# mpkuse/rgbd_odometry

Measured on AMD Instinct MI355X. Metric: frame-pair aligns/sec (640x480, 4-lvl pyr), higher is better.
Workload: dtype f32

## Files before the change

### rgbd_odometry_amd/csrc/dvo_fused.hip

```cpp
#include "dvo_kernel_common.h"
#include "dvo_point_pk.h"
#include "dvo_palette.h"
#include "dvo_tiled_step.h"

#include <type_traits>

#ifndef DVO_WPE256
#define DVO_WPE256 2
#endif
#ifndef DVO_P4_DEPTH
#define DVO_P4_DEPTH(BLOCK) ((BLOCK) == 256 ? 3 : 2)
#endif

namespace dvo {

template <bool WITH_H, bool WITH_E2 = false>
struct Acc7T {
    static constexpr bool with_h = WITH_H, with_e2 = WITH_E2;
    double g[6];
    double e2;
    int nvis;
    double H[WITH_H ? 21 : 1];
    E2Limbs l;
};
typedef Acc7T<false> Acc7;

template <typename ACC>
DVO_DEV void acc7_zero(ACC &a) {
#pragma unroll
    for (int k = 0; k < 6; k++) a.g[k] = 0.0;
    a.e2 = 0.0;
    a.nvis = 0;
    if constexpr (ACC::with_h) {
#pragma unroll
        for (int k = 0; k < 21; k++) a.H[k] = 0.0;
    }
    if constexpr (ACC::with_e2) e2_limbs_zero(a.l);
}
template <typename ACC>
DVO_DEV void acc_h_add(ACC &a, const double *jwd, const double *Jd) {
#pragma unroll
    for (int i = 0; i < 6; i++)
#pragma unroll
        for (int j = i; j < 6; j++) a.H[i * 6 - (i * (i - 1)) / 2 + (j - i)] = fma(jwd[i], Jd[j], a.H[i * 6 - (i * (i - 1)) / 2 + (j - i)]);
}

enum { TEX_G16 = DVO_TEXMODE_GLOBAL16, TEX_L16 = DVO_TEXMODE_LDS16, TEX_P4 = DVO_TEXMODE_PAL4 };

struct TexSrc {
    const char *g16;
    unsigned tile_col_bytes;
    const char *l16;
    const char *p4;
    unsigned p4_col_bytes;
};

struct __attribute__((packed, aligned(4))) U3 { unsigned a, b, c; };

template <int TEX> struct Round2 {
    v2f xn, yn, zn;
    v4f t0, t1;
    bool vis0, vis1;
};
template <> struct Round2<TEX_P4> {
    v2f xn, yn, zn;
    U3 t0, t1;
};

typedef const __attribute__((address_space(3))) float lds_cfloat;
typedef const __attribute__((address_space(3))) v2f lds_cv2f;

DVO_DEV unsigned texel_byte_offset(int yy, int xx, unsigned tile_col_bytes ) {
    static_assert(DVO_TILE_Y_LOG2 == 2 && DVO_TILE_X_LOG2 == 1, "written for 4x2 tiles");
    return __umul24((unsigned)(xx >> 1), tile_col_bytes) + ((unsigned)yy << 5) - (((unsigned)yy & 3u) << 4) + (((unsigned)xx & 1u) << 6);
}

DVO_DEV unsigned p4_byte_offset(int yy, int xx, unsigned p4_col_bytes ) {
    static_assert(DVO_P4_ROWS == 6, "written for 6 interior rows per line");
    const unsigned ty = __umul24((unsigned)yy, 43691u) >> 18;
    return __umul24((unsigned)(xx >> 2), p4_col_bytes) + 128u  + (((unsigned)xx & 3u) << 5) + ((unsigned)yy << 2) + __umul24(ty, 104u);
}

struct LdsPoints {
    const uint2 *p;
    const unsigned *w4;
    const unsigned *g4;
    const unsigned *hdr;
};

template <bool LDS_SRC>
DVO_DEV void load_compact(const LdsPoints &lp, const uint2 *__restrict__ gpts, int j, unsigned &k, float &z) {
    const uint2 a = LDS_SRC ? lp.p[j] : gpts[j];
    k = a.x; z = __uint_as_float(a.y);
}

struct PointPf { uint2 p0, p1; unsigned h0, h1;  };

DVO_DEV unsigned pt4_header(const LdsPoints &lp, int i, int end) {
    const int chunk = __builtin_amdgcn_readfirstlane(min(i, end - 1)) >> 6;
    return lp.hdr[chunk];
}
struct PointPf4 { unsigned w0, w1; };

DVO_DEV uint2 stream_point(const uint2 *__restrict__ p) { return *p; }
DVO_DEV unsigned stream_word(const unsigned *__restrict__ p) { return *p; }
template <bool LDS_SRC, int TEX, bool PT4 = false, bool FULL = false>
DVO_DEV void round2_issue(const IterConst &c, const TexSrc &ts, const LdsPoints &lp, const uint2 *__restrict__ gpts,
                          int i0, int i1, int end, int step, PointPf &pf, Round2<TEX> &b, bool &any_odd, int &nvis) {
    const bool valid0 = FULL || i0 < end, valid1 = FULL || i1 < end;
    v2f xx, yy, Z;
    if constexpr (PT4) {
        unsigned w0, w1;
        if constexpr (LDS_SRC) {
            w0 = lp.w4[valid0 ? i0 : (end - 1)];
            w1 = lp.w4[valid1 ? i1 : (end - 1)];
        } else {
            w0 = pf.p0.x; w1 = pf.p1.x;
            pf.p0.x = stream_word(lp.g4 + min(i0 + step, end - 1));
            pf.p1.x = stream_word(lp.g4 + min(i1 + step, end - 1));
        }
        float x0, y0, z0, x1, y1, z1;
        const unsigned L00 = pf.h0, L01 = pf.h1;
        pf.h0 = pt4_header(lp, i0 + step, end);
        pf.h1 = pt4_header(lp, i1 + step, end);
        pt4_decode(c.nby, c.inv_nby, c.half_inv_nby, w0, L00, x0, y0, z0);
        pt4_decode(c.nby, c.inv_nby, c.half_inv_nby, w1, L01, x1, y1, z1);
        xx.x = x0; xx.y = x1; yy.x = y0; yy.y = y1; Z.x = z0; Z.y = z1;
    } else {
    unsigned k0, k1;
    float z0, z1;
    if constexpr (LDS_SRC) {
        const int j0 = valid0 ? i0 : (end - 1), j1 = valid1 ? i1 : (end - 1);
        load_compact<true>(lp, gpts, j0, k0, z0);
        load_compact<true>(lp, gpts, j1, k1, z1);
    } else {
        k0 = pf.p0.x; z0 = __uint_as_float(pf.p0.y);
        k1 = pf.p1.x; z1 = __uint_as_float(pf.p1.y);
        pf.p0 = stream_point(gpts + min(i0 + step, end - 1));
        pf.p1 = stream_point(gpts + min(i1 + step, end - 1));
    }
    xx.x = (float)(k0 & 0xffffu); xx.y = (float)(k1 & 0xffffu);
    yy.x = (float)(k0 >> 16);     yy.y = (float)(k1 >> 16);
    Z.x = z0; Z.y = z1;
    }
    const v2f X = (Z * (xx - c.pcx)) * c.pfx;
    const v2f Y = (Z * (yy - c.pcy)) * c.pfy;
    v2f xn, yn, zn, u, v;
    if constexpr (TEX == TEX_P4) {
        lanemask odd;
        project_point2m(c, X, Y, Z, xn, yn, zn, u, v, odd);
        any_odd |= (odd != 0ull);
        int px0, py0, px1, py1;
        const lanemask in0 = pixel_in_range_mask(u.x, c.cols, px0) & pixel_in_range_mask(v.x, c.rows, py0);
        const lanemask in1 = pixel_in_range_mask(u.y, c.cols, px1) & pixel_in_range_mask(v.y, c.rows, py1);
        const lanemask vis0 = FULL ? in0 : (in0 & mask_lt_i32(i0, end)), vis1 = FULL ? in1 : (in1 & mask_lt_i32(i1, end));
        b.xn = xn; b.yn = yn; b.zn = zn;
        nvis += __popcll(vis0) + __popcll(vis1);
        const unsigned o0 = select_or_zero(vis0, p4_byte_offset(py0, px0, ts.p4_col_bytes));
        const unsigned o1 = select_or_zero(vis1, p4_byte_offset(py1, px1, ts.p4_col_bytes));
        b.t0 = *reinterpret_cast<const U3 *>(ts.p4 + o0);
        b.t1 = *reinterpret_cast<const U3 *>(ts.p4 + o1);
    } else {
        bool odd0, odd1;
        project_point2(c, X, Y, Z, xn, yn, zn, u, v, odd0, odd1);
        any_odd |= (__builtin_amdgcn_ballot_w64(odd0 || odd1) != 0ull);
        int px0, py0, px1, py1;
        const bool inx0 = pixel_in_range(u.x, c.cols, px0), iny0 = pixel_in_range(v.x, c.rows, py0);
        const bool inx1 = pixel_in_range(u.y, c.cols, px1), iny1 = pixel_in_range(v.y, c.rows, py1);
        const bool vis0 = inx0 && iny0 && valid0;
        const bool vis1 = inx1 && iny1 && valid1;
        b.xn = xn; b.yn = yn; b.zn = zn;
        b.vis0 = vis0; b.vis1 = vis1;
        unsigned o0 = texel_byte_offset(py0, px0, ts.tile_col_bytes);
        unsigned o1 = texel_byte_offset(py1, px1, ts.tile_col_bytes);
        o0 = vis0 ? o0 : 0u;
        o1 = vis1 ? o1 : 0u;
        const char *base = (TEX == TEX_L16) ? ts.l16 : ts.g16;
        b.t0 = *reinterpret_cast<const v4f *>(base + o0);
        b.t1 = *reinterpret_cast<const v4f *>(base + o1);
    }
}

DVO_DEV unsigned lshl3_add(int d, unsigned c) {
    unsigned r;
    asm("v_lshl_add_u32 %0, %1, 3, %2" : "=v"(r) : "v"(d), "v"(c));
    return r;
}
template <unsigned PAL>
DVO_DEV void p4_decode2(const U3 &t0, const U3 &t1, v2f &dt, v2f &gx, v2f &gy, v2f &w) {
    const unsigned c0 = t0.b & 0xfff8u, c1 = t1.b & 0xfff8u;
    const v2f pw0 = *(lds_cv2f *)(size_t)(PAL + c0);
    const v2f pw1 = *(lds_cv2f *)(size_t)(PAL + c1);
    v2f pu, pd, pr, pl;
    pu.x = *(lds_cfloat *)(size_t)(PAL + (t0.a & 0xfff8u));
    pu.y = *(lds_cfloat *)(size_t)(PAL + (t1.a & 0xfff8u));
    pd.x = *(lds_cfloat *)(size_t)(PAL + (t0.c & 0xfff8u));
    pd.y = *(lds_cfloat *)(size_t)(PAL + (t1.c & 0xfff8u));
    pr.x = *(lds_cfloat *)(size_t)(PAL + lshl3_add(__builtin_amdgcn_sbfe((int)t0.b, 16, 8), c0));
    pr.y = *(lds_cfloat *)(size_t)(PAL + lshl3_add(__builtin_amdgcn_sbfe((int)t1.b, 16, 8), c1));
    pl.x = *(lds_cfloat *)(size_t)(PAL + lshl3_add(((int)t0.b) >> 24, c0));
    pl.y = *(lds_cfloat *)(size_t)(PAL + lshl3_add(((int)t1.b) >> 24, c1));
    dt.x = pw0.x; dt.y = pw1.x; w.x = pw0.y; w.y = pw1.y;
    gx = (pr - pl) * 0.5f;
    gy = (pd - pu) * 0.5f;
}

template <typename ACC>
DVO_DEV void acc7_add(ACC &a, const float *jw, const float *J, float eps) {
    const double e = (double)eps;
    double jwd[6];
#pragma unroll
    for (int k = 0; k < 6; k++) { jwd[k] = (double)jw[k]; a.g[k] = fma(jwd[k], e, a.g[k]); }
    a.e2 = fma(e, e, a.e2);
    if constexpr (ACC::with_e2) e2_limbs_add(a.l, eps);
    if constexpr (ACC::with_h) {
        double Jd[6];
#pragma unroll
        for (int k = 0; k < 6; k++) Jd[k] = (double)J[k];
        acc_h_add(a, jwd, Jd);
    }
}

DVO_DEV void iter_const_pose(IterConst &c, const float *Rf, const float *tf) {
    c.r[0] = uniform_f(Rf[0]); c.r[1] = uniform_f(Rf[1]); c.r[2] = uniform_f(Rf[2]);
    c.r[3] = uniform_f(Rf[3]); c.r[4] = uniform_f(Rf[4]); c.r[5] = uniform_f(Rf[5]);
    c.r[6] = uniform_f(Rf[6]); c.r[7] = uniform_f(Rf[7]); c.r[8] = uniform_f(Rf[8]);
    c.t[0] = uniform_f(tf[0]); c.t[1] = uniform_f(tf[1]); c.t[2] = uniform_f(tf[2]);
}

struct AccE2 {
    static constexpr bool with_h = false;
    E2Limbs l;
    int nvis;
};
DVO_DEV void acc7_add(AccE2 &a, const float *, const float *, float eps) { e2_limbs_add(a.l, eps); }

template <int TEX, unsigned PAL, typename ACC>
DVO_DEV void round2_compute(const IterConst &c, const Round2<TEX> &b, ACC &a) {
    v2f jw[6], J[6];
    float eps0, eps1;
    if constexpr (TEX == TEX_P4) {
        v2f dt, gx, gy, wt;
        p4_decode2<PAL>(b.t0, b.t1, dt, gx, gy, wt);
        eps0 = dt.x; eps1 = dt.y;
        jacobian_weighted2p(c, b.xn, b.yn, b.zn, gx, gy, wt, jw, ACC::with_h ? J : nullptr);
    } else {
        a.nvis += __popcll(__builtin_amdgcn_ballot_w64(b.vis0)) + __popcll(__builtin_amdgcn_ballot_w64(b.vis1));
        eps0 = b.vis0 ? b.t0.x : 0.0f; eps1 = b.vis1 ? b.t1.x : 0.0f;
        const float w0 = b.vis0 ? b.t0.w : 0.0f, w1 = b.vis1 ? b.t1.w : 0.0f;
        const float gx0 = b.vis0 ? b.t0.y : 0.0f, gx1 = b.vis1 ? b.t1.y : 0.0f;
        const float gy0 = b.vis0 ? b.t0.z : 0.0f, gy1 = b.vis1 ? b.t1.z : 0.0f;
        jacobian_weighted2(c, b.xn, b.yn, b.zn, gx0, gx1, gy0, gy1, w0, w1, jw, ACC::with_h ? J : nullptr);
    }
    const double e0 = (double)eps0, e1 = (double)eps1;
    if constexpr (ACC::with_e2) { e2_limbs_add(a.l, eps0); e2_limbs_add(a.l, eps1); }
    if constexpr (!ACC::with_h) {
#pragma unroll
        for (int k = 0; k < 6; k++) {
            a.g[k] = fma((double)jw[k].x, e0, a.g[k]);
            a.g[k] = fma((double)jw[k].y, e1, a.g[k]);
        }
        a.e2 = fma(e0, e0, a.e2);
        a.e2 = fma(e1, e1, a.e2);
    } else {
        {
            double jd[6], Jd[6];
#pragma unroll
            for (int k = 0; k < 6; k++) { jd[k] = (double)jw[k].x; Jd[k] = (double)J[k].x; a.g[k] = fma(jd[k], e0, a.g[k]); }
            a.e2 = fma(e0, e0, a.e2);
            acc_h_add(a, jd, Jd);
        }
        __builtin_amdgcn_sched_barrier(0);
        {
            double jd[6], Jd[6];
#pragma unroll
            for (int k = 0; k < 6; k++) { jd[k] = (double)jw[k].y; Jd[k] = (double)J[k].y; a.g[k] = fma(jd[k], e1, a.g[k]); }
            a.e2 = fma(e1, e1, a.e2);
            acc_h_add(a, jd, Jd);
        }
        __builtin_amdgcn_sched_barrier(0);
    }
}

template <int BLOCK, bool LDS_SRC, int TEX, int DEPTH = 2, unsigned PAL = 0, bool PT4 = false, typename ACC = Acc7>
DVO_DEV void accumulate_points2(const IterConst &c, const TexSrc &ts, const LdsPoints &lp, const uint2 *__restrict__ gpts,
                                int first, int end, int lane_off, ACC &a, bool &any_odd) {
    if (first >= end) return;
    constexpr int STEP = 2 * BLOCK;
    const int wave_off = __builtin_amdgcn_readfirstlane(lane_off - (int)(threadIdx.x & 63));
    const int n_rounds = (end - first - wave_off + STEP - 1) / STEP;
    if (n_rounds <= 0) return;
#define DVO_ISSUE(buf, k) round2_issue<LDS_SRC, TEX, PT4>(c, ts, lp, gpts, base + (k) * STEP, base + (k) * STEP + BLOCK, end, STEP, pf, buf, any_odd, a.nvis)
#define DVO_ISSUE_FULL(buf, k) round2_issue<LDS_SRC, TEX, PT4, true>(c, ts, lp, gpts, base + (k) * STEP, base + (k) * STEP + BLOCK, end, STEP, pf, buf, any_odd, a.nvis)
#define DVO_COMPUTE(buf) round2_compute<TEX, PAL, ACC>(c, buf, a)
    int base = first + lane_off;
    PointPf pf;
    if constexpr (PT4) { pf.h0 = pt4_header(lp, base, end); pf.h1 = pt4_header(lp, base + BLOCK, end); }
    if constexpr (!LDS_SRC) {
        if constexpr (PT4) { pf.p0.x = stream_word(lp.g4 + min(base, end - 1)); pf.p1.x = stream_word(lp.g4 + min(base + BLOCK, end - 1)); }
        else { pf.p0 = stream_point(gpts + min(base, end - 1)); pf.p1 = stream_point(gpts + min(base + BLOCK, end - 1)); }
    }
    if constexpr (DEPTH == 3) {
        Round2<TEX> A, B, C;
        DVO_ISSUE(A, 0);
        if (n_rounds > 1) DVO_ISSUE(B, 1);
        int r = 0;
        for (; r + 4 < n_rounds; r += 3) {
            DVO_ISSUE_FULL(C, 2); DVO_COMPUTE(A);
            DVO_ISSUE_FULL(A, 3); DVO_COMPUTE(B);
            DVO_ISSUE(B, 4); DVO_COMPUTE(C);
            base += 3 * STEP;
        }
        const int left = n_rounds - r;
        if (left >= 3) DVO_ISSUE(C, 2);
        DVO_COMPUTE(A);
        if (left >= 2) {
            if (left >= 4) DVO_ISSUE(A, 3);
            DVO_COMPUTE(B);
            if (left >= 3) {
                DVO_COMPUTE(C);
                if (left >= 4) DVO_COMPUTE(A);
            }
        }
    } else {
        Round2<TEX> A, B;
        DVO_ISSUE(A, 0);
        int r = 0;
        for (; r + 2 < n_rounds; r += 2) {
            DVO_ISSUE_FULL(B, 1); DVO_COMPUTE(A);
            DVO_ISSUE(A, 2); DVO_COMPUTE(B);
            base += 2 * STEP;
        }
        if (r + 1 < n_rounds) {
            DVO_ISSUE(B, 1);
            DVO_COMPUTE(A);
            DVO_COMPUTE(B);
        } else {
            DVO_COMPUTE(A);
        }
    }
#undef DVO_ISSUE
#undef DVO_ISSUE_FULL
#undef DVO_COMPUTE
}

DVO_DEV float4 p4_texel(const TexSrc &ts, const float2 *pal_lds, int yy, int xx) {
    const U3 w = *reinterpret_cast<const U3 *>(ts.p4 + p4_byte_offset(yy, xx, ts.p4_col_bytes));
    const int c = (int)((w.b >> 3) & 0x1fffu);
    const int cr = c + __builtin_amdgcn_sbfe((int)w.b, 16, 8), cl = c + (((int)w.b) >> 24);
    const float2 pc = pal_lds[c];
    const float pr = pal_lds[cr].x, pl = pal_lds[cl].x, pu = pal_lds[(w.a >> 3) & 0x1fffu].x, pd = pal_lds[(w.c >> 3) & 0x1fffu].x;
    return make_float4(pc.x, (pr - pl) * 0.5f, (pd - pu) * 0.5f, pc.y);
}

template <int BLOCK, bool LDS_SRC, bool P4, bool PT4 = false, typename ACC = Acc7>
DVO_DEV void accumulate_points_exact(const IterConst &c, const char *__restrict__ tex, const TexSrc &ts, const float2 *pal_lds,
                                     const LdsPoints &lp, const uint2 *__restrict__ gpts, int first, int end, int lane_off, ACC &a) {
    for (int i = first + lane_off; __builtin_amdgcn_ballot_w64(i < end) != 0ull; i += BLOCK) {
        const bool valid = i < end;
        float X, Y, Z, xn, yn, zn, u, v;
        if constexpr (PT4) {
            const int j = valid ? i : (end - 1);
            const unsigned w = LDS_SRC ? lp.w4[j] : lp.g4[j];
            float xf, yf;
            pt4_decode(c.nby, c.inv_nby, c.half_inv_nby, w, pt4_header(lp, i, end), xf, yf, Z);
            X = Z * (xf - c.pcx) * c.pfx;
            Y = Z * (yf - c.pcy) * c.pfy;
        } else {
        unsigned k; float z;
        load_compact<LDS_SRC>(lp, gpts, valid ? i : (end - 1), k, z);
        expand_compact(c, k, z, X, Y, Z);
        }
        const bool vis = project_point(c, X, Y, Z, xn, yn, zn, u, v) && valid;
        a.nvis += __popcll(__builtin_amdgcn_ballot_w64(vis));
        if (vis) {
            const float4 t = P4 ? p4_texel(ts, pal_lds, (int)v, (int)u)
                                : reinterpret_cast<const float4 *>(tex)[texel_index((int)v, (int)u, c.tiles_per_col)];
            float J[6], jw[6];
            jacobian_row(c, xn, yn, zn, t.y, t.z, J);
#pragma unroll
            for (int q = 0; q < 6; q++) jw[q] = J[q] * t.w;
            acc7_add(a, jw, J, t.x);
        }
    }
}

template <int BLOCK, typename ACC>
DVO_DEV void sweep_literal(int mode, bool p4_partial, bool pt4, const IterConst &c, const char *__restrict__ tex, const TexSrc &ts, const float2 *pal_lds,
                           const LdsPoints &lp, const uint2 *__restrict__ gpts, int n_lds, int N, int lane_off, ACC &a) {
    if (mode == DVO_TEXMODE_PAL4 && p4_partial && pt4) {
        accumulate_points_exact<BLOCK, true, false, true, ACC>(c, tex, ts, pal_lds, lp, gpts, 0, n_lds, lane_off, a);
        accumulate_points_exact<BLOCK, false, false, true, ACC>(c, tex, ts, pal_lds, lp, gpts, n_lds, N, lane_off, a);
    } else if (mode == DVO_TEXMODE_PAL4 && p4_partial) {
        accumulate_points_exact<BLOCK, true, false, false, ACC>(c, tex, ts, pal_lds, lp, gpts, 0, n_lds, lane_off, a);
        accumulate_points_exact<BLOCK, false, false, false, ACC>(c, tex, ts, pal_lds, lp, gpts, n_lds, N, lane_off, a);
    } else if (mode == DVO_TEXMODE_PAL4 && pt4) {
        accumulate_points_exact<BLOCK, true, true, true, ACC>(c, tex, ts, pal_lds, lp, gpts, 0, n_lds, lane_off, a);
        accumulate_points_exact<BLOCK, false, true, true, ACC>(c, tex, ts, pal_lds, lp, gpts, n_lds, N, lane_off, a);
    } else if (mode == DVO_TEXMODE_PAL4) {
        accumulate_points_exact<BLOCK, true, true, false, ACC>(c, tex, ts, pal_lds, lp, gpts, 0, n_lds, lane_off, a);
        accumulate_points_exact<BLOCK, false, true, false, ACC>(c, tex, ts, pal_lds, lp, gpts, n_lds, N, lane_off, a);
    } else {
        accumulate_points_exact<BLOCK, true, false, false, ACC>(c, tex, ts, pal_lds, lp, gpts, 0, n_lds, lane_off, a);
        accumulate_points_exact<BLOCK, false, false, false, ACC>(c, tex, ts, pal_lds, lp, gpts, n_lds, N, lane_off, a);
    }
}

struct Final2 {
    v2f u, v, zn;
    unsigned w0, w1;
    bool vis0, vis1;
};
template <bool LDS_SRC, int TEX, bool PT4 = false>
DVO_DEV void final2_issue(const IterConst &c, const TexSrc &ts, const LdsPoints &lp, const uint2 *__restrict__ gpts,
                          int i0, int i1, int end, int step, PointPf &pf, Final2 &b) {
    float X0, Y0, Z0, X1, Y1, Z1;
    if constexpr (PT4) {
        unsigned w0, w1;
        if constexpr (LDS_SRC) {
            w0 = lp.w4[min(i0, end - 1)]; w1 = lp.w4[min(i1, end - 1)];
        } else {
            w0 = pf.p0.x; w1 = pf.p1.x;
            pf.p0.x = stream_word(lp.g4 + min(i0 + step, end - 1));
            pf.p1.x = stream_word(lp.g4 + min(i1 + step, end - 1));
        }
        float xf, yf;
        pt4_decode(c.nby, c.inv_nby, c.half_inv_nby, w0, pt4_header(lp, i0, end), xf, yf, Z0);
        X0 = Z0 * (xf - c.pcx) * c.pfx; Y0 = Z0 * (yf - c.pcy) * c.pfy;
        pt4_decode(c.nby, c.inv_nby, c.half_inv_nby, w1, pt4_header(lp, i1, end), xf, yf, Z1);
        X1 = Z1 * (xf - c.pcx) * c.pfx; Y1 = Z1 * (yf - c.pcy) * c.pfy;
    } else {
        unsigned k0, k1;
        float z0, z1;
        if constexpr (LDS_SRC) {
            load_compact<true>(lp, gpts, min(i0, end - 1), k0, z0);
            load_compact<true>(lp, gpts, min(i1, end - 1), k1, z1);
        } else {
            k0 = pf.p0.x; z0 = __uint_as_float(pf.p0.y);
            k1 = pf.p1.x; z1 = __uint_as_float(pf.p1.y);
            pf.p0 = stream_point(gpts + min(i0 + step, end - 1));
            pf.p1 = stream_point(gpts + min(i1 + step, end - 1));
        }
        expand_compact(c, k0, z0, X0, Y0, Z0);
        expand_compact(c, k1, z1, X1, Y1, Z1);
    }
    {
        float xs, ys, zs, us, vs;
        project_point(c, X0, Y0, Z0, xs, ys, zs, us, vs);
        b.u.x = us; b.v.x = vs; b.zn.x = zs;
        project_point(c, X1, Y1, Z1, xs, ys, zs, us, vs);
        b.u.y = us; b.v.y = vs; b.zn.y = zs;
    }
    int px0, py0, px1, py1;
    const bool inx0 = pixel_in_range(b.u.x, c.cols, px0), iny0 = pixel_in_range(b.v.x, c.rows, py0);
    const bool inx1 = pixel_in_range(b.u.y, c.cols, px1), iny1 = pixel_in_range(b.v.y, c.rows, py1);
    b.vis0 = inx0 && iny0; b.vis1 = inx1 && iny1;
    if constexpr (TEX == TEX_P4) {
        const unsigned o0 = b.vis0 ? p4_byte_offset(py0, px0, ts.p4_col_bytes) + 4u : 0u;
        const unsigned o1 = b.vis1 ? p4_byte_offset(py1, px1, ts.p4_col_bytes) + 4u : 0u;
        b.w0 = *reinterpret_cast<const unsigned *>(ts.p4 + o0);
        b.w1 = *reinterpret_cast<const unsigned *>(ts.p4 + o1);
    } else {
        const unsigned o0 = b.vis0 ? texel_byte_offset(py0, px0, ts.tile_col_bytes) : 0u;
        const unsigned o1 = b.vis1 ? texel_byte_offset(py1, px1, ts.tile_col_bytes) : 0u;
        const char *base = (TEX == TEX_L16) ? ts.l16 : ts.g16;
        b.w0 = *reinterpret_cast<const unsigned *>(base + o0);
        b.w1 = *reinterpret_cast<const unsigned *>(base + o1);
    }
}
template <int TEX, unsigned PAL>
DVO_DEV void final2_store(const Final2 &b, int i0, int i1, int end, float *__restrict__ fe, float *__restrict__ fr, const TexSrc &ts, bool partial) {
    float e0, e1;
    if constexpr (TEX == TEX_P4) {
        e0 = *(lds_cfloat *)(size_t)(PAL + (b.w0 & 0xfff8u));
        e1 = *(lds_cfloat *)(size_t)(PAL + (b.w1 & 0xfff8u));
        if (partial && __builtin_amdgcn_ballot_w64((e0 != e0) || (e1 != e1)) != 0ull) {
            if (e0 != e0) e0 = *reinterpret_cast<const float *>(ts.g16 + texel_byte_offset((int)b.v.x, (int)b.u.x, ts.tile_col_bytes));
            if (e1 != e1) e1 = *reinterpret_cast<const float *>(ts.g16 + texel_byte_offset((int)b.v.y, (int)b.u.y, ts.tile_col_bytes));
// ... 194 lines not shown
    }
    auto team_total = [&](double sl) -> double {
        v4u *tb = reinterpret_cast<v4u *>(out.team_buf);
        if (super_team) {
            sl = team_exchange(sl, tb + (size_t)xcd * 2 * DVO_TEAM_MAX * 8, local, G >> 3, epoch, out.team_err, true, team_same_xcd);
            return team_exchange(sl, tb + (size_t)8 * 2 * DVO_TEAM_MAX * 8, xcd, 8, epoch, out.team_err, local == 0);
        }
        return team_exchange(sl, tb + (size_t)pair_local * 2 * DVO_TEAM_MAX * 8, member, G, epoch, out.team_err, true, team_same_xcd);
    };
    static_assert(BLOCK >= 128, "wave 0 runs the update, wave 1 the bookkeeping");
    constexpr unsigned kPose = (unsigned)((sizeof(PoseState) + 15) & ~15u);
    constexpr unsigned kRedH = WITH_H ? (BLOCK / 64) * 24 * 8 : 0;
    constexpr unsigned kStatic = kPose + (BLOCK / 64) * 64 + 64 + kRedH;
    __shared__ __attribute__((aligned(16))) char s_static[kStatic];
    double (*const redH)[24] = reinterpret_cast<double (*)[24]>(s_static + kPose + (BLOCK / 64) * 64 + 64);
    PoseState &st = *reinterpret_cast<PoseState *>(s_static);
    double (*const red)[8] = reinterpret_cast<double (*)[8]>(s_static + kPose);
    double *const tot = reinterpret_cast<double *>(s_static + kPose + (BLOCK / 64) * 64);
    UpdConst &uc = st.u;
    extern __shared__ __attribute__((aligned(16))) float lds_dyn[];
    const bool pal_base_ok = (unsigned)(size_t)(__attribute__((address_space(3))) float *)lds_dyn == kStatic;

    if (tid == 0) {
        const double *p = out.poses + (size_t)pair * 12;
        const bool ident = (sc.flags & 2) != 0;
        double R0[9], t0[3];
#pragma unroll
        for (int k = 0; k < 9; k++) R0[k] = ident ? ((k % 4 == 0) ? 1.0 : 0.0) : p[k];
#pragma unroll
        for (int k = 0; k < 3; k++) t0[k] = ident ? 0.0 : p[9 + k];
        pose_state_load(st, R0, t0);
        upd_const_build(uc, prm);
    }
    __syncthreads();

    for (int l = sc.n_levels - 1; l >= 0; --l) {
        const int iters = sc.iters[l];
        if (iters <= 0) continue;
        const LevelSlab &L = lv.l[l];
        const int dpair = (sc.alias_mod > 0) ? (pair % sc.alias_mod) : pair;
        const int Nall = __builtin_amdgcn_readfirstlane(L.N[dpair]);
        int pfirst = 0, N = Nall;
        if (TEAM) {
            const int chunk = (((Nall + G - 1) / G) + 1) & ~1;
            pfirst = min(Nall, member * chunk);
            N = min(Nall, pfirst + chunk) - pfirst;
        }
        const char *__restrict__ tex = reinterpret_cast<const char *>(L.tex + (size_t)dpair * L.tex_stride);
        const uint2 *__restrict__ gpts = L.cpts + (size_t)dpair * L.pt_cap + pfirst;
        float *energy = out.energy + (size_t)pair * sc.e_stride + sc.e_off[l];

        IterConst c;
        level_consts(c, WITH_H ? K : pair_intrinsics(K, dpair), l, L.rows, L.cols);

        if (member == 0)
            for (int i = tid; i < iters; i += BLOCK) energy[i] = 0.0f;
        if (tid == 0) { pose_state_begin(st); pose_regulariser_precompute(st, st.p[0], uc); }

        const int lds_words = sc.lds_bytes >> 2;
        const int n_pad = (N + 3) & ~3;
        const int tex16_words = (int)(L.tex_stride * 4);
        const int pal_n_raw = (!sc.no_p4 && L.pal_n) ? __builtin_amdgcn_readfirstlane(L.pal_n[dpair]) : 0;
        const int n_pal = pal_count(pal_n_raw);
        const bool p4_partial = pal_partial(pal_n_raw);
        const int mode = (n_pal > 0 && pal_base_ok && 2 * n_pal + 8 <= lds_words) ? TEX_P4
                         : ((!TEAM && !sc.no_lds_tex && 2 * n_pad + tex16_words <= lds_words) ? TEX_L16 : TEX_G16);
        const int n_pal_lds = n_pal + (p4_partial ? 2 : 1);
        const int pal_words = (mode == TEX_P4) ? ((2 * n_pal_lds + 3) & ~3) : 0;
        const bool pt4 = !TEAM && mode == TEX_P4 && !sc.no_pt4 && N >= (((lds_words - pal_words) >> 1) & ~1) && L.pt4_ok &&
                         __builtin_amdgcn_readfirstlane(L.pt4_ok[dpair]) != 0;
        float *const lds_pts = lds_dyn + pal_words;
        const int cap = (mode == TEX_L16) ? n_pad
                        : (pt4 ? ((lds_words - pal_words) & ~1) : (((lds_words - pal_words) >> 1) & ~1));
        const int n_lds = (N <= cap) ? N : (cap / (2 * BLOCK)) * (2 * BLOCK);
        float *const lds_tex = lds_pts + 2 * cap;
        if (tid == 0) { st.exact_ran = 0; st.e2_open = 0; st.e2_ran = 0; }
        if (mode == TEX_P4) {
            const float2 *__restrict__ pg = L.pal + (size_t)dpair * DVO_PAL_MAX;
            float2 *pl = reinterpret_cast<float2 *>(lds_dyn);
            for (int i = tid; i < n_pal_lds; i += BLOCK) pl[i] = pg[i];
        }
        const unsigned *__restrict__ g4pts = L.cpt4 + (size_t)dpair * L.pt_cap + pfirst;
        if (pt4) {
            const uint4 *g4 = reinterpret_cast<const uint4 *>(g4pts);
            uint4 *d4 = reinterpret_cast<uint4 *>(lds_pts);
            const int n4 = n_lds >> 2;
            int i = tid;
            for (; i + 3 * BLOCK < n4; i += 4 * BLOCK) {
                uint4 v[4];
#pragma unroll
                for (int q = 0; q < 4; q++) v[q] = g4[i + q * BLOCK];
#pragma unroll
                for (int q = 0; q < 4; q++) d4[i + q * BLOCK] = v[q];
            }
            for (; i < n4; i += BLOCK) d4[i] = g4[i];
            for (int j = (n4 << 2) + tid; j < n_lds; j += BLOCK) reinterpret_cast<unsigned *>(lds_pts)[j] = g4pts[j];
        } else {
            const uint4 *g4 = reinterpret_cast<const uint4 *>(gpts);
            uint4 *d4 = reinterpret_cast<uint4 *>(lds_pts);
            const int n2 = n_lds >> 1;
            int i = tid;
            for (; i + 3 * BLOCK < n2; i += 4 * BLOCK) {
                uint4 v[4];
#pragma unroll
                for (int q = 0; q < 4; q++) v[q] = g4[i + q * BLOCK];
#pragma unroll
                for (int q = 0; q < 4; q++) d4[i + q * BLOCK] = v[q];
            }
            for (; i < n2; i += BLOCK) d4[i] = g4[i];
            if ((n_lds & 1) && tid == 0) reinterpret_cast<uint2 *>(lds_pts)[n_lds - 1] = gpts[n_lds - 1];
        }
        if (mode == TEX_L16) {
            const v4f *g = reinterpret_cast<const v4f *>(tex);
            v4f *d = reinterpret_cast<v4f *>(lds_tex);
            const int n16 = (int)L.tex_stride;
            int i = tid;
            for (; i + 3 * BLOCK < n16; i += 4 * BLOCK) {
                v4f v[4];
#pragma unroll
                for (int q = 0; q < 4; q++) v[q] = g[i + q * BLOCK];
#pragma unroll
                for (int q = 0; q < 4; q++) d[i + q * BLOCK] = v[q];
            }
            for (; i < n16; i += BLOCK) d[i] = g[i];
        }
        LdsPoints lp;
        lp.p = reinterpret_cast<const uint2 *>(lds_pts);
        lp.w4 = reinterpret_cast<const unsigned *>(lds_pts);
        lp.g4 = g4pts;
        lp.hdr = L.chdr + (size_t)dpair * (L.pt_cap >> 6);
        TexSrc ts;
        ts.g16 = tex; ts.tile_col_bytes = (unsigned)c.tiles_per_col * 128u;
        ts.l16 = reinterpret_cast<const char *>(lds_tex);
        ts.p4 = reinterpret_cast<const char *>(L.p4 + (size_t)dpair * L.p4_stride);
        ts.p4_col_bytes = (unsigned)p4_tiles_per_col(L.rows) * 128u;
        __syncthreads();

        const bool exch = TEAM;
        for (int itr = 0; itr < iters; ++itr) {
            if (!TEAM) {
                if (l > 0) __builtin_amdgcn_s_setprio(3);
                else if (2 * itr < iters) __builtin_amdgcn_s_setprio(2);
                else if (4 * itr < 3 * iters) __builtin_amdgcn_s_setprio(1);
                else __builtin_amdgcn_s_setprio(0);
            }
            const PoseCur &pc = st.p[itr & 1];
            PoseCur &pn = st.p[(itr + 1) & 1];
            iter_const_pose(c, pc.Rf, pc.tf);

            Acc7T<WITH_H> a;
            acc7_zero(a);
            bool any_odd = false;
            const int lane_off = BLOCK - 64 - (tid & ~63) + (tid & 63);
            if (mode == TEX_L16) {
                accumulate_points2<BLOCK, true, TEX_L16, 2, 0, false, Acc7T<WITH_H>>(c, ts, lp, gpts, 0, N, lane_off, a, any_odd);
            } else if (mode == TEX_P4 && pt4) {
                accumulate_points2<BLOCK, true, TEX_P4, (WITH_H ? 2 : DVO_P4_DEPTH(BLOCK)), kStatic, true, Acc7T<WITH_H>>(c, ts, lp, gpts, 0, n_lds, lane_off, a, any_odd);
                accumulate_points2<BLOCK, false, TEX_P4, (WITH_H ? 2 : DVO_P4_DEPTH(BLOCK)), kStatic, true, Acc7T<WITH_H>>(c, ts, lp, gpts, n_lds, N, lane_off, a, any_odd);
            } else if (mode == TEX_P4) {
                accumulate_points2<BLOCK, true, TEX_P4, (WITH_H ? 2 : DVO_P4_DEPTH(BLOCK)), kStatic, false, Acc7T<WITH_H>>(c, ts, lp, gpts, 0, n_lds, lane_off, a, any_odd);
                accumulate_points2<BLOCK, false, TEX_P4, (WITH_H ? 2 : DVO_P4_DEPTH(BLOCK)), kStatic, false, Acc7T<WITH_H>>(c, ts, lp, gpts, n_lds, N, lane_off, a, any_odd);
            } else {
                accumulate_points2<BLOCK, true, TEX_G16, 2, 0, false, Acc7T<WITH_H>>(c, ts, lp, gpts, 0, n_lds, lane_off, a, any_odd);
                accumulate_points2<BLOCK, false, TEX_G16, 2, 0, false, Acc7T<WITH_H>>(c, ts, lp, gpts, n_lds, N, lane_off, a, any_odd);
            }
            {
                const double chk = ((a.g[0] + a.g[1]) + (a.g[2] + a.g[3])) + ((a.g[4] + a.g[5]) + a.e2);
                any_odd |= (__builtin_amdgcn_ballot_w64(!__builtin_isfinite(chk)) != 0ull);
            }
            if (any_odd || sc.force_exact) {
                acc7_zero(a);
                sweep_literal<BLOCK>(mode, p4_partial, pt4, c, tex, ts, reinterpret_cast<const float2 *>(lds_dyn), lp, gpts, n_lds, N, lane_off, a);
                if ((tid & 63) == 0) st.exact_ran = 1;
            }
            wave_sums7(a, red);
            if constexpr (WITH_H) {
#pragma unroll
                for (int q = 0; q < 3; q++) {
                    double d[8];
#pragma unroll
                    for (int k = 0; k < 8; k++) d[k] = (8 * q + k < 21) ? a.H[8 * q + k] : 0.0;
                    wave_reduce_scatter8_dpp(d);
                    const int idx = reduce_scatter8_dpp_index(tid & 63);
                    if ((tid & 63) < 8) redH[tid >> 6][8 * q + idx] = d[0];
                }
            }
            const int wave = __builtin_amdgcn_readfirstlane(tid >> 6), lane = tid & 63;
            double neg_step = 0.0;
            if (wave == 0) neg_step = pose_neg_step(uc, itr);
            __syncthreads();
            double sl = 0.0;
            if (wave == 0) {
                sl = block_sum8<BLOCK>(red, lane & 7);
                if (exch) {
                    sl = team_total(sl);
                    if (lane == 6 || lane == 7) tot[lane] = sl;
                }
            }
            if (exch) __syncthreads();
            if (wave == 0) {
                double psi[6];
                pose_direction_lanes(st, uc, neg_step, sl, lane, psi);
                if (lane == 0) pose_apply(st, pc, pn, uc, psi);
            } else if (WITH_H && wave == 2) {
                if (lane < 21) {
                    double hs = 0.0;
#pragma unroll
                    for (int w = 0; w < BLOCK / 64; w++) hs += redH[w][lane];
                    out.H[((size_t)pair * sc.e_stride + sc.e_off[l] + itr) * 21 + lane] = hs;
                }
            } else if (wave == 1 && lane == 0) {
                const double e2 = exch ? tot[6] : block_sum8<BLOCK>(red, 6);
                const double nv = exch ? tot[7] : block_sum8<BLOCK>(red, 7);
                float e;
                if (energy_certified(e2, Nall, e) && !sc.force_e2) {
                    pose_bookkeep_e(st, pc, itr, Nall, e, (int)nv);
                    if (member == 0) energy[itr] = e;
                } else {
                    st.e2_fast = e2;
                    st.e2_nvis = (int)nv;
                    st.e2_open = 1;
                }
            }
            if (exch) epoch++;
            __syncthreads();
            if (st.e2_open) {
                AccE2 ae;
                e2_limbs_zero(ae.l);
                ae.nvis = 0;
                sweep_literal<BLOCK>(mode, p4_partial, pt4, c, tex, ts, reinterpret_cast<const float2 *>(lds_dyn), lp, gpts, n_lds, N, lane_off, ae);
                wave_sums_e2(ae, red);
                __syncthreads();
                if (wave == 0) {
                    double sl2 = block_sum8<BLOCK>(red, lane & 7);
                    if (exch) sl2 = team_total(sl2);
                    if (lane < 3) tot[lane] = sl2;
                }
                if (exch) epoch++;
                __syncthreads();
                if (wave == 1 && lane == 0) {
                    const float e = (float)sqrt(e2_from_limbs(tot[0], tot[1], tot[2], st.e2_fast));
                    pose_bookkeep_e(st, pc, itr, Nall, e, st.e2_nvis);
                    if (member == 0) energy[itr] = e;
                    st.e2_open = 0;
                    st.e2_ran++;
                }
                __syncthreads();
            }
            if (st.stop) break;
            if (tid == 0 && itr + 1 < iters) pose_regulariser_precompute(st, pn, uc);
        }

        if ((sc.flags & 1) && l == sc.last_level) {
            if (st.bestItr >= 0) {
                iter_const_pose(c, st.bRf, st.btf);
                float *fe = out.final_eps + (size_t)pair * out.final_cap;
                float *fr = out.final_reproj + (size_t)pair * out.final_cap * 3;
                float *fes = fe + pfirst, *frs = fr + 3 * (size_t)pfirst;
#ifndef DVO_NO_FINAL
                if (mode == TEX_P4 && pt4) {
                    final_outputs2<BLOCK, true, TEX_P4, kStatic, true>(c, ts, lp, gpts, 0, n_lds, fes, frs, p4_partial);
                    final_outputs2<BLOCK, false, TEX_P4, kStatic, true>(c, ts, lp, gpts, n_lds, N, fes, frs, p4_partial);
                } else if (mode == TEX_P4) {
                    final_outputs2<BLOCK, true, TEX_P4, kStatic>(c, ts, lp, gpts, 0, n_lds, fes, frs, p4_partial);
                    final_outputs2<BLOCK, false, TEX_P4, kStatic>(c, ts, lp, gpts, n_lds, N, fes, frs, p4_partial);
                } else if (mode == TEX_L16) {
                    final_outputs2<BLOCK, true, TEX_L16, kStatic>(c, ts, lp, gpts, 0, N, fes, frs);
                } else {
                    final_outputs2<BLOCK, true, TEX_G16, kStatic>(c, ts, lp, gpts, 0, n_lds, fes, frs);
                    final_outputs2<BLOCK, false, TEX_G16, kStatic>(c, ts, lp, gpts, n_lds, N, fes, frs);
                }
#endif
            }
            if (tid == 0 && member == 0) out.final_N[pair] = (st.bestItr >= 0) ? Nall : 0;
        }
        __syncthreads();
        if (tid == 0) {
            pose_state_finish(st);
            if (member == 0) {
                out.best_idx[pair * DVO_LEVELS + l] = st.bestItr;
                out.ratio[pair * DVO_LEVELS + l] = st.bestRatio;
                out.tex_mode[pair * DVO_LEVELS + l] = mode | (st.exact_ran ? DVO_TEXMODE_EXACT_RAN : 0) | (pt4 ? DVO_TEXMODE_PT4 : 0) |
                                                       (min(st.e2_ran, DVO_TEXMODE_E2_MAX) << DVO_TEXMODE_E2_SHIFT);
            }
        }
        __syncthreads();
    }

    if (tid == 0 && member == 0) {
        double *p = out.poses + (size_t)pair * 12;
#pragma unroll
        for (int k = 0; k < 9; k++) p[k] = st.R[k];
#pragma unroll
        for (int k = 0; k < 3; k++) p[9 + k] = st.p[0].t[k];
    }
}

template <int BLOCK>
static hipError_t launch_fused2_b(const LevelSet &lv, const Schedule &sc, const Intrinsics &K, const DevParams &prm,
                                  const Outputs &out, int first_pair, int n_pairs, hipStream_t s) {
    const size_t dyn = (size_t)sc.lds_bytes;
    hipError_t e;
    if constexpr (BLOCK == 512) {
        if (sc.flags & 4) {
            if (sc.team > 1 || !out.H) return hipErrorInvalidValue;
            auto kern = align_fused2_kernel<512, false, true>;
            if ((e = hipFuncSetAttribute((const void *)kern, hipFuncAttributeMaxDynamicSharedMemorySize, (int)dyn)) != hipSuccess) return e;
            hipLaunchKernelGGL(kern, dim3(n_pairs), dim3(512), dyn, s, lv, sc, K, prm, out, first_pair);
            return hipGetLastError();
        }
    } else if constexpr (BLOCK == 256) {
        if (sc.flags & 4) {
            if (sc.team > 1 || !out.H) return hipErrorInvalidValue;
            auto kern = align_fused2_kernel<256, false, true>;
            if ((e = hipFuncSetAttribute((const void *)kern, hipFuncAttributeMaxDynamicSharedMemorySize, (int)dyn)) != hipSuccess) return e;
            hipLaunchKernelGGL(kern, dim3(n_pairs), dim3(256), dyn, s, lv, sc, K, prm, out, first_pair);
            return hipGetLastError();
        }
    } else {
        if (sc.flags & 4) return hipErrorInvalidValue;
    }
    if (sc.team > 1) {
        auto kern = align_fused2_kernel<BLOCK, true>;
        if ((e = hipFuncSetAttribute((const void *)kern, hipFuncAttributeMaxDynamicSharedMemorySize, (int)dyn)) != hipSuccess) return e;
        const int grid = (sc.team > DVO_TEAM_MAX) ? sc.team : 8 * ((n_pairs + 7) / 8) * sc.team;
        {
            struct Seen { int dev = -1; size_t dyn = 0; long long limit = 0; };
            thread_local Seen seen;
            int dev = 0;
            if ((e = hipGetDevice(&dev)) != hipSuccess) return e;
            if (seen.dev != dev || seen.dyn != dyn) {
                int per_cu = 0, n_cu = 0;
                if ((e = hipOccupancyMaxActiveBlocksPerMultiprocessor(&per_cu, (const void *)kern, BLOCK, dyn)) != hipSuccess) return e;
                if ((e = hipDeviceGetAttribute(&n_cu, hipDeviceAttributeMultiprocessorCount, dev)) != hipSuccess) return e;
                seen.dev = dev; seen.dyn = dyn; seen.limit = (long long)per_cu * n_cu;
            }
            if ((long long)grid > seen.limit) return hipErrorCooperativeLaunchTooLarge;
        }
        hipLaunchKernelGGL(kern, dim3(grid), dim3(BLOCK), dyn, s, lv, sc, K, prm, out, first_pair);
    } else {
        auto kern = align_fused2_kernel<BLOCK, false>;
        if ((e = hipFuncSetAttribute((const void *)kern, hipFuncAttributeMaxDynamicSharedMemorySize, (int)dyn)) != hipSuccess) return e;
        hipLaunchKernelGGL(kern, dim3(n_pairs), dim3(BLOCK), dyn, s, lv, sc, K, prm, out, first_pair);
    }
    return hipGetLastError();
}

size_t fused2_static_lds(int block_threads, bool with_h) {
    return ((sizeof(PoseState) + 15) & ~(size_t)15) + (size_t)(block_threads / 64) * 64 + 64 + (with_h ? (size_t)(block_threads / 64) * 24 * 8 : 0) + 16;
}

hipError_t launch_align_fused2(int block_threads, const LevelSet &lv, const Schedule &sc, const Intrinsics &K,
                               const DevParams &prm, const Outputs &out, int first_pair, int n_pairs, hipStream_t s) {
    if (n_pairs <= 0) return hipSuccess;
    if (sc.team > DVO_TEAM_MAX && !(n_pairs == 1 && (sc.team == 64 || sc.team == 128 || sc.team == 256))) return hipErrorInvalidValue;
    switch (block_threads) {
// ... 172 lines not shown
```

Measured before the change: 792,900.

## Use residual-only accumulation pass on final iteration without gradient or pose update

On the last iteration of the non-Hessian path, the kernel now runs a specialised accumulation that loads only the residual texel word and accumulates the squared error, skipping gradient and Jacobian work. The pose direction and pose update are also skipped on that iteration, since their result would not be used. This reduces memory traffic and ALU work for one pass out of each level's iterations. The cost is extra template instantiations, more code size, and a second code path that must stay consistent with the exact sweep fallback.

```diff
diff --git a/rgbd_odometry_amd/csrc/dvo_fused.hip b/rgbd_odometry_amd/csrc/dvo_fused.hip
--- a/rgbd_odometry_amd/csrc/dvo_fused.hip
+++ b/rgbd_odometry_amd/csrc/dvo_fused.hip
@@ -10,6 +10,9 @@
 #endif
 #ifndef DVO_P4_DEPTH
 #define DVO_P4_DEPTH(BLOCK) ((BLOCK) == 256 ? 3 : 2)
+#endif
+#ifndef DVO_P4_DEPTH_E
+#define DVO_P4_DEPTH_E(BLOCK) DVO_P4_DEPTH(BLOCK)
 #endif
 
 namespace dvo {
@@ -58,14 +61,33 @@
 struct __attribute__((packed, aligned(4))) U3 { unsigned a, b, c; };
 
 template <int TEX> struct Round2 {
+    static constexpr bool residual_only = false;
     v2f xn, yn, zn;
     v4f t0, t1;
     bool vis0, vis1;
 };
 template <> struct Round2<TEX_P4> {
+    static constexpr bool residual_only = false;
     v2f xn, yn, zn;
     U3 t0, t1;
 };
+
+template <int TEX> struct RoundE {
+    static constexpr bool residual_only = true;
+    float d0, d1;
+    bool vis0, vis1;
+};
+template <> struct RoundE<TEX_P4> {
+    static constexpr bool residual_only = true;
+    unsigned w0, w1;
+};
+struct AccR {
+    static constexpr bool with_h = false, with_e2 = false, residual_only = true;
+    double e2;
+    int nvis;
+};
+template <int TEX, typename ACC> struct RoundOf { typedef Round2<TEX> type; };
+template <int TEX> struct RoundOf<TEX, AccR> { typedef RoundE<TEX> type; };
 
 typedef const __attribute__((address_space(3))) float lds_cfloat;
 typedef const __attribute__((address_space(3))) v2f lds_cv2f;
@@ -104,9 +126,9 @@
 
 DVO_DEV uint2 stream_point(const uint2 *__restrict__ p) { return *p; }
 DVO_DEV unsigned stream_word(const unsigned *__restrict__ p) { return *p; }
-template <bool LDS_SRC, int TEX, bool PT4 = false, bool FULL = false>
+template <bool LDS_SRC, int TEX, bool PT4 = false, bool FULL = false, typename BUF >
 DVO_DEV void round2_issue(const IterConst &c, const TexSrc &ts, const LdsPoints &lp, const uint2 *__restrict__ gpts,
-                          int i0, int i1, int end, int step, PointPf &pf, Round2<TEX> &b, bool &any_odd, int &nvis) {
+                          int i0, int i1, int end, int step, PointPf &pf, BUF &b, bool &any_odd, int &nvis) {
     const bool valid0 = FULL || i0 < end, valid1 = FULL || i1 < end;
     v2f xx, yy, Z;
     if constexpr (PT4) {
@@ -154,12 +176,17 @@
         const lanemask in0 = pixel_in_range_mask(u.x, c.cols, px0) & pixel_in_range_mask(v.x, c.rows, py0);
         const lanemask in1 = pixel_in_range_mask(u.y, c.cols, px1) & pixel_in_range_mask(v.y, c.rows, py1);
         const lanemask vis0 = FULL ? in0 : (in0 & mask_lt_i32(i0, end)), vis1 = FULL ? in1 : (in1 & mask_lt_i32(i1, end));
-        b.xn = xn; b.yn = yn; b.zn = zn;
         nvis += __popcll(vis0) + __popcll(vis1);
         const unsigned o0 = select_or_zero(vis0, p4_byte_offset(py0, px0, ts.p4_col_bytes));
         const unsigned o1 = select_or_zero(vis1, p4_byte_offset(py1, px1, ts.p4_col_bytes));
-        b.t0 = *reinterpret_cast<const U3 *>(ts.p4 + o0);
-        b.t1 = *reinterpret_cast<const U3 *>(ts.p4 + o1);
+        if constexpr (BUF::residual_only) {
+            b.w0 = *reinterpret_cast<const unsigned *>(ts.p4 + 4 + o0);
+            b.w1 = *reinterpret_cast<const unsigned *>(ts.p4 + 4 + o1);
+        } else {
+            b.xn = xn; b.yn = yn; b.zn = zn;
+            b.t0 = *reinterpret_cast<const U3 *>(ts.p4 + o0);
+            b.t1 = *reinterpret_cast<const U3 *>(ts.p4 + o1);
+        }
     } else {
         bool odd0, odd1;
         project_point2(c, X, Y, Z, xn, yn, zn, u, v, odd0, odd1);
@@ -169,15 +196,20 @@
         const bool inx1 = pixel_in_range(u.y, c.cols, px1), iny1 = pixel_in_range(v.y, c.rows, py1);
         const bool vis0 = inx0 && iny0 && valid0;
         const bool vis1 = inx1 && iny1 && valid1;
-        b.xn = xn; b.yn = yn; b.zn = zn;
         b.vis0 = vis0; b.vis1 = vis1;
         unsigned o0 = texel_byte_offset(py0, px0, ts.tile_col_bytes);
         unsigned o1 = texel_byte_offset(py1, px1, ts.tile_col_bytes);
         o0 = vis0 ? o0 : 0u;
         o1 = vis1 ? o1 : 0u;
         const char *base = (TEX == TEX_L16) ? ts.l16 : ts.g16;
-        b.t0 = *reinterpret_cast<const v4f *>(base + o0);
-        b.t1 = *reinterpret_cast<const v4f *>(base + o1);
+        if constexpr (BUF::residual_only) {
+            b.d0 = *reinterpret_cast<const float *>(base + o0);
+            b.d1 = *reinterpret_cast<const float *>(base + o1);
+        } else {
+            b.xn = xn; b.yn = yn; b.zn = zn;
+            b.t0 = *reinterpret_cast<const v4f *>(base + o0);
+            b.t1 = *reinterpret_cast<const v4f *>(base + o1);
+        }
     }
 }
 
@@ -234,6 +266,10 @@
     int nvis;
 };
 DVO_DEV void acc7_add(AccE2 &a, const float *, const float *, float eps) { e2_limbs_add(a.l, eps); }
+DVO_DEV void acc7_add(AccR &a, const float *, const float *, float eps) {
+    const double e = (double)eps;
+    a.e2 = fma(e, e, a.e2);
+}
 
 template <int TEX, unsigned PAL, typename ACC>
 DVO_DEV void round2_compute(const IterConst &c, const Round2<TEX> &b, ACC &a) {
@@ -280,6 +316,21 @@
         }
         __builtin_amdgcn_sched_barrier(0);
     }
+}
+
+template <int TEX, unsigned PAL>
+DVO_DEV void round2_compute(const IterConst &, const RoundE<TEX> &b, AccR &a) {
+    float eps0, eps1;
+    if constexpr (TEX == TEX_P4) {
+        eps0 = *(lds_cfloat *)(size_t)(PAL + (b.w0 & 0xfff8u));
+        eps1 = *(lds_cfloat *)(size_t)(PAL + (b.w1 & 0xfff8u));
+    } else {
+        a.nvis += __popcll(__builtin_amdgcn_ballot_w64(b.vis0)) + __popcll(__builtin_amdgcn_ballot_w64(b.vis1));
+        eps0 = b.vis0 ? b.d0 : 0.0f; eps1 = b.vis1 ? b.d1 : 0.0f;
+    }
+    const double e0 = (double)eps0, e1 = (double)eps1;
+    a.e2 = fma(e0, e0, a.e2);
+    a.e2 = fma(e1, e1, a.e2);
 }
 
 template <int BLOCK, bool LDS_SRC, int TEX, int DEPTH = 2, unsigned PAL = 0, bool PT4 = false, typename ACC = Acc7>
@@ -292,7 +343,7 @@
     if (n_rounds <= 0) return;
 #define DVO_ISSUE(buf, k) round2_issue<LDS_SRC, TEX, PT4>(c, ts, lp, gpts, base + (k) * STEP, base + (k) * STEP + BLOCK, end, STEP, pf, buf, any_odd, a.nvis)
 #define DVO_ISSUE_FULL(buf, k) round2_issue<LDS_SRC, TEX, PT4, true>(c, ts, lp, gpts, base + (k) * STEP, base + (k) * STEP + BLOCK, end, STEP, pf, buf, any_odd, a.nvis)
-#define DVO_COMPUTE(buf) round2_compute<TEX, PAL, ACC>(c, buf, a)
+#define DVO_COMPUTE(buf) round2_compute<TEX, PAL>(c, buf, a)
     int base = first + lane_off;
     PointPf pf;
     if constexpr (PT4) { pf.h0 = pt4_header(lp, base, end); pf.h1 = pt4_header(lp, base + BLOCK, end); }
@@ -301,7 +352,7 @@
         else { pf.p0 = stream_point(gpts + min(base, end - 1)); pf.p1 = stream_point(gpts + min(base + BLOCK, end - 1)); }
     }
     if constexpr (DEPTH == 3) {
-        Round2<TEX> A, B, C;
+        typename RoundOf<TEX, ACC>::type A, B, C;
         DVO_ISSUE(A, 0);
         if (n_rounds > 1) DVO_ISSUE(B, 1);
         int r = 0;
@@ -323,7 +374,7 @@
             }
         }
     } else {
-        Round2<TEX> A, B;
+        typename RoundOf<TEX, ACC>::type A, B;
         DVO_ISSUE(A, 0);
         int r = 0;
         for (; r + 2 < n_rounds; r += 2) {
@@ -824,26 +875,53 @@
             acc7_zero(a);
             bool any_odd = false;
             const int lane_off = BLOCK - 64 - (tid & ~63) + (tid & 63);
-            if (mode == TEX_L16) {
-                accumulate_points2<BLOCK, true, TEX_L16, 2, 0, false, Acc7T<WITH_H>>(c, ts, lp, gpts, 0, N, lane_off, a, any_odd);
-            } else if (mode == TEX_P4 && pt4) {
-                accumulate_points2<BLOCK, true, TEX_P4, (WITH_H ? 2 : DVO_P4_DEPTH(BLOCK)), kStatic, true, Acc7T<WITH_H>>(c, ts, lp, gpts, 0, n_lds, lane_off, a, any_odd);
-                accumulate_points2<BLOCK, false, TEX_P4, (WITH_H ? 2 : DVO_P4_DEPTH(BLOCK)), kStatic, true, Acc7T<WITH_H>>(c, ts, lp, gpts, n_lds, N, lane_off, a, any_odd);
-            } else if (mode == TEX_P4) {
-                accumulate_points2<BLOCK, true, TEX_P4, (WITH_H ? 2 : DVO_P4_DEPTH(BLOCK)), kStatic, false, Acc7T<WITH_H>>(c, ts, lp, gpts, 0, n_lds, lane_off, a, any_odd);
-                accumulate_points2<BLOCK, false, TEX_P4, (WITH_H ? 2 : DVO_P4_DEPTH(BLOCK)), kStatic, false, Acc7T<WITH_H>>(c, ts, lp, gpts, n_lds, N, lane_off, a, any_odd);
+            const bool last = !WITH_H && itr == iters - 1;
+            if (last) {
+                if constexpr (!WITH_H) {
+                    AccR ar;
+                    ar.e2 = 0.0; ar.nvis = 0;
+                    if (mode == TEX_L16) {
+                        accumulate_points2<BLOCK, true, TEX_L16, 2, 0, false, AccR>(c, ts, lp, gpts, 0, N, lane_off, ar, any_odd);
+                    } else if (mode == TEX_P4 && pt4) {
+                        accumulate_points2<BLOCK, true, TEX_P4, DVO_P4_DEPTH_E(BLOCK), kStatic, true, AccR>(c, ts, lp, gpts, 0, n_lds, lane_off, ar, any_odd);
+                        accumulate_points2<BLOCK, false, TEX_P4, DVO_P4_DEPTH_E(BLOCK), kStatic, true, AccR>(c, ts, lp, gpts, n_lds, N, lane_off, ar, any_odd);
+                    } else if (mode == TEX_P4) {
+                        accumulate_points2<BLOCK, true, TEX_P4, DVO_P4_DEPTH_E(BLOCK), kStatic, false, AccR>(c, ts, lp, gpts, 0, n_lds, lane_off, ar, any_odd);
+                        accumulate_points2<BLOCK, false, TEX_P4, DVO_P4_DEPTH_E(BLOCK), kStatic, false, AccR>(c, ts, lp, gpts, n_lds, N, lane_off, ar, any_odd);
+                    } else {
+                        accumulate_points2<BLOCK, true, TEX_G16, 2, 0, false, AccR>(c, ts, lp, gpts, 0, n_lds, lane_off, ar, any_odd);
+                        accumulate_points2<BLOCK, false, TEX_G16, 2, 0, false, AccR>(c, ts, lp, gpts, n_lds, N, lane_off, ar, any_odd);
+                    }
+                    any_odd |= (__builtin_amdgcn_ballot_w64(!__builtin_isfinite(ar.e2)) != 0ull);
+                    if (any_odd || sc.force_exact) {
+                        ar.e2 = 0.0; ar.nvis = 0;
+                        sweep_literal<BLOCK>(mode, p4_partial, pt4, c, tex, ts, reinterpret_cast<const float2 *>(lds_dyn), lp, gpts, n_lds, N, lane_off, ar);
+                        if ((tid & 63) == 0) st.exact_ran = 1;
+                    }
+                    a.e2 = ar.e2; a.nvis = ar.nvis;
+                }
             } else {
-                accumulate_points2<BLOCK, true, TEX_G16, 2, 0, false, Acc7T<WITH_H>>(c, ts, lp, gpts, 0, n_lds, lane_off, a, any_odd);
-                accumulate_points2<BLOCK, false, TEX_G16, 2, 0, false, Acc7T<WITH_H>>(c, ts, lp, gpts, n_lds, N, lane_off, a, any_odd);
-            }
-            {
-                const double chk = ((a.g[0] + a.g[1]) + (a.g[2] + a.g[3])) + ((a.g[4] + a.g[5]) + a.e2);
-                any_odd |= (__builtin_amdgcn_ballot_w64(!__builtin_isfinite(chk)) != 0ull);
-            }
-            if (any_odd || sc.force_exact) {
-                acc7_zero(a);
-                sweep_literal<BLOCK>(mode, p4_partial, pt4, c, tex, ts, reinterpret_cast<const float2 *>(lds_dyn), lp, gpts, n_lds, N, lane_off, a);
-                if ((tid & 63) == 0) st.exact_ran = 1;
+                if (mode == TEX_L16) {
+                    accumulate_points2<BLOCK, true, TEX_L16, 2, 0, false, Acc7T<WITH_H>>(c, ts, lp, gpts, 0, N, lane_off, a, any_odd);
+                } else if (mode == TEX_P4 && pt4) {
+                    accumulate_points2<BLOCK, true, TEX_P4, (WITH_H ? 2 : DVO_P4_DEPTH(BLOCK)), kStatic, true, Acc7T<WITH_H>>(c, ts, lp, gpts, 0, n_lds, lane_off, a, any_odd);
+                    accumulate_points2<BLOCK, false, TEX_P4, (WITH_H ? 2 : DVO_P4_DEPTH(BLOCK)), kStatic, true, Acc7T<WITH_H>>(c, ts, lp, gpts, n_lds, N, lane_off, a, any_odd);
+                } else if (mode == TEX_P4) {
+                    accumulate_points2<BLOCK, true, TEX_P4, (WITH_H ? 2 : DVO_P4_DEPTH(BLOCK)), kStatic, false, Acc7T<WITH_H>>(c, ts, lp, gpts, 0, n_lds, lane_off, a, any_odd);
+                    accumulate_points2<BLOCK, false, TEX_P4, (WITH_H ? 2 : DVO_P4_DEPTH(BLOCK)), kStatic, false, Acc7T<WITH_H>>(c, ts, lp, gpts, n_lds, N, lane_off, a, any_odd);
+                } else {
+                    accumulate_points2<BLOCK, true, TEX_G16, 2, 0, false, Acc7T<WITH_H>>(c, ts, lp, gpts, 0, n_lds, lane_off, a, any_odd);
+                    accumulate_points2<BLOCK, false, TEX_G16, 2, 0, false, Acc7T<WITH_H>>(c, ts, lp, gpts, n_lds, N, lane_off, a, any_odd);
+                }
+                {
+                    const double chk = ((a.g[0] + a.g[1]) + (a.g[2] + a.g[3])) + ((a.g[4] + a.g[5]) + a.e2);
+                    any_odd |= (__builtin_amdgcn_ballot_w64(!__builtin_isfinite(chk)) != 0ull);
+                }
+                if (any_odd || sc.force_exact) {
+                    acc7_zero(a);
+                    sweep_literal<BLOCK>(mode, p4_partial, pt4, c, tex, ts, reinterpret_cast<const float2 *>(lds_dyn), lp, gpts, n_lds, N, lane_off, a);
+                    if ((tid & 63) == 0) st.exact_ran = 1;
+                }
             }
             wave_sums7(a, red);
             if constexpr (WITH_H) {
@@ -871,9 +949,11 @@
             }
             if (exch) __syncthreads();
             if (wave == 0) {
-                double psi[6];
-                pose_direction_lanes(st, uc, neg_step, sl, lane, psi);
-                if (lane == 0) pose_apply(st, pc, pn, uc, psi);
+                if (!last) {
+                    double psi[6];
+                    pose_direction_lanes(st, uc, neg_step, sl, lane, psi);
+                    if (lane == 0) pose_apply(st, pc, pn, uc, psi);
+                }
             } else if (WITH_H && wave == 2) {
                 if (lane < 21) {
                     double hs = 0.0;
```

Measured after the change: 808,600 (median of 6 runs). 1.02x the previous value.
